# microsoft/UniVL

Measured on NVIDIA H100. Metric: video-text samples/sec, higher is better.
Workload: dtype bf16

## Files before the change

include/univl_b200.h:

```cpp
#ifndef UNIVL_B200_H_
#define UNIVL_B200_H_

#ifdef __cplusplus
extern "C" {
#endif

const char* univl_last_error_string(void);
int univl_abi_version(void);
int univl_set_reserved_sms(int n);

int univl_gemm_bf16(const void* A, long long lda, int a_mn_major, const void* B, long long ldb, int b_mn_major,
                    int M, int N, int Kc, void* out, long long ldo, int epilogue, const float* bias,
                    const void* aux_in, long long ld_aux_in, void* aux_out, long long ld_aux_out, float alpha,
                    int block_n, int split_k, void* stream);
int univl_gemm_plan(int M, int N, int Kc, int epilogue, int block_n, int split_k);

int univl_quantize_e4m3_rows(const void* x, long long ldx, void* q, long long ldq, float* scale, int M, int K,
                             void* stream);
int univl_quantize_e4m3_blocks(const float* w, long long ldw, void* q, long long ldq, float* scale, int N, int K,
                               void* stream);
int univl_gemm_fp8(const void* A, long long lda, const float* a_scale, const void* B, long long ldb,
                   const float* b_scale, int M, int N, int Kc, int epilogue, const float* bias, void* out,
                   long long ldo, float* out_scale, void* stream);

int univl_layernorm_fwd(const void* x, const void* res, const float* gamma, const float* beta, void* y, float* mean,
                        float* rstd, int rows, int cols, float eps, float p_drop, int drop_mode,
                        const unsigned long long* rng_state, unsigned long long stream_id, void* stream);
int univl_layernorm_bwd(const void* dy, const void* dy2, const void* x, const void* res, const float* gamma,
                        const float* mean, const float* rstd, void* dx_res, void* dx_dense, float* dgamma,
                        float* dbeta, float* dbias, int rows, int cols, float p_drop, int drop_mode,
                        const unsigned long long* rng_state, unsigned long long stream_id, void* stream);
int univl_layernorm_f32_fwd(const float* x, const float* gamma, const float* beta, void* y, float* mean, float* rstd,
                            int rows, int cols, float eps, void* stream);
int univl_layernorm_f32_bwd(const void* dy, const float* x, const float* gamma, const float* mean, const float* rstd,
                            float* dgamma, float* dbeta, int rows, int cols, void* stream);

int univl_embed_text_fwd(const long long* ids, const long long* type_ids, const float* word, const float* pos,
                         const float* type, const float* gamma, const float* beta, void* y, float* mean, float* rstd,
                         int n_seq, int S, int H, int vocab, float eps, float p_drop, const unsigned long long* rng_state,
                         unsigned long long stream_id, void* stream);
int univl_embed_text_bwd(const void* dy, const long long* ids, const long long* type_ids, const float* word,
                         const float* pos, const float* type, const float* gamma, const float* mean,
                         const float* rstd, float* dword, float* dpos, float* dtype, float* dgamma, float* dbeta,
                         int n_seq, int S, int H, int vocab, float p_drop, const unsigned long long* rng_state,
                         unsigned long long stream_id, void* stream);
int univl_embed_src_fwd(const void* a, const void* b, const float* pos, const float* type, const float* gamma,
                        const float* beta, void* y, float* mean, float* rstd, int Na, int Wa, int Nb, int Fb,
                        int all_pairs, int H, float eps, float p_drop, const unsigned long long* rng_state,
                        unsigned long long stream_id, void* stream);
int univl_embed_src_bwd(const void* dy, const void* a, const void* b, const float* pos, const float* type,
                        const float* gamma, const float* mean, const float* rstd, void* da, void* db, float* dpos,
                        float* dtype, float* dgamma, float* dbeta, int Na, int Wa, int Nb, int Fb, int all_pairs,
                        int H, float p_drop, const unsigned long long* rng_state, unsigned long long stream_id, void* stream);

int univl_attention_fwd(const void* q, long long ldq, const void* k, long long ldk, const void* v, long long ldv,
                        void* o, long long ldo, float* lse, const long long* mask_a, const long long* mask_b, int Wa,
                        int Fb, int Nb, int all_pairs, int n_seq, int heads, int Sq, int Sk, int causal, float scale,
                        float p_drop, const unsigned long long* rng_state, unsigned long long stream_id, void* stream);
int univl_attention_bwd(const void* q, long long ldq, const void* k, long long ldk, const void* v, long long ldv,
                        const void* o, long long ldo, const float* lse, const void* d_o, long long lddo, void* dq,
                        long long lddq, void* dk, long long lddk, void* dv, long long lddv, const long long* mask_a,
                        const long long* mask_b, int Wa, int Fb, int Nb, int all_pairs, int n_seq, int heads, int Sq,
                        int Sk, int causal, float scale, float p_drop, const unsigned long long* rng_state,
                        unsigned long long stream_id, int rng_layout, float* dbq, float* dbk, float* dbv, void* stream);
int univl_attention_long_fwd(const void* q, long long ldq, const void* k, long long ldk, const void* v, long long ldv,
                             void* o, long long ldo, float* lse, const long long* mask_a, const long long* mask_b,
                             int Wa, int Fb, int Nb, int all_pairs, int n_seq, int heads, int Sq, int Sk, int causal,
                             float scale, float p_drop, const unsigned long long* rng_state,
                             unsigned long long stream_id, void* stream);
int univl_attention_long_bwd(const void* q, long long ldq, const void* k, long long ldk, const void* v, long long ldv,
                             const void* o, long long ldo, const float* lse, const void* d_o, long long lddo, void* dq,
                             long long lddq, void* dk, long long lddk, void* dv, long long lddv,
                             const long long* mask_a, const long long* mask_b, int Wa, int Fb, int Nb, int all_pairs,
                             int n_seq, int heads, int Sq, int Sk, int causal, float scale, float p_drop,
                             const unsigned long long* rng_state, unsigned long long stream_id, int rng_layout,
                             float* dbq, float* dbk, float* dbv, void* stream);
int univl_attention_pair_fwd(const void* qa, long long ldqa, const void* ka, long long ldka, const void* va,
                             long long ldva, const void* qb, long long ldqb, const void* kb, long long ldkb,
                             const void* vb, long long ldvb, void* o, long long ldo, float* lse,
                             const long long* mask_a, const long long* mask_b, int Na, int Wa, int Nb, int Fb,
                             int heads, int Sq, float scale, void* stream);
int univl_fused_qkv_attention_supported(int n_seq, int heads, int S, int H);
int univl_fused_qkv_attention_fwd(const void* x, long long ldx, const void* wqkv, long long ldw, const float* bias,
                                  void* qkv_out, long long ld_qkv, void* o, long long ldo, float* lse,
                                  const long long* mask_a, const long long* mask_b, int Wa, int Fb, int Nb,
                                  int all_pairs, int n_seq, int heads, int S, int causal, float scale, float p_drop,
                                  const unsigned long long* rng_state, unsigned long long stream_id, void* stream);
int univl_fused_attention_bwd(const void* qkv, long long ld_qkv, const void* o, long long ldo, const float* lse,
                              const void* d_o, long long lddo, void* dqkv, long long ld_dqkv, float* dbias,
                              const long long* mask_a, const long long* mask_b, int Wa, int Fb, int Nb, int all_pairs,
                              int n_seq, int heads, int S, int causal, float scale, float p_drop,
                              const unsigned long long* rng_state, unsigned long long stream_id, void* stream);

int univl_colsum_bf16(const void* x, long long ld, float* out, int rows, int cols, void* stream);
int univl_cast_f32_to_bf16(const float* src, void* dst, long long n, void* stream);
int univl_cast_bf16_to_f32(const void* src, float* dst, long long n, void* stream);
int univl_multi_cast_f32_to_bf16(const unsigned long long* device_table, int n_tensors, int blocks_per_tensor,
                                 void* stream);
int univl_fill_f32(float* p, float value, long long n, void* stream);
int univl_rng_advance(unsigned long long* rng_state, void* stream);
int univl_gelu_fwd_bf16(const void* x, void* out, long long n, void* stream);
int univl_gelu_bwd_bf16(const void* dy, const void* pre, void* out, long long n, void* stream);
int univl_tanh_fwd_bf16(const void* x, void* out, long long n, void* stream);
int univl_tanh_bwd_bf16(const void* dy, const void* y, void* out, long long n, void* stream);
int univl_scale_f32(float* dst, const float* src, long long n, const float* gscale, void* stream);

int univl_meanpool_fwd(const void* x, const long long* mask, float* out, float* norm_out, int N, int S, int H,
                       int skip_first, int guard_zero, int l2norm, void* stream);
int univl_meanpool_bwd(const float* dy, const float* y, const float* norm, const long long* mask, void* dx, int N,
                       int S, int H, int skip_first, int guard_zero, int l2norm, void* stream);
int univl_sim_matmul_fwd(const float* t, const float* v, float* sim, int Bt, int Bv, int H, int groups, void* stream);
int univl_sim_matmul_bwd(const float* dsim, const float* t, const float* v, float* dt, float* dv, int Bt, int Bv,
                         int H, int groups, void* stream);
int univl_maxmargin_loss(const float* sim, float* loss, float* dsim, int B, float margin, int n_pair, float w_same,
                         float w_diff, int groups, void* stream);
int univl_crossen_loss(const float* sim, float* loss, float* dsim, int B, int groups, void* stream);
int univl_milnce_loss(const float* sim, float* loss, float* dsim, int batch_size, int n_pair, int groups,
                      void* stream);
int univl_softmax_xent_fwd(const float* logits, long long ld, const long long* labels, const long long* pair_mask,
                           float* lse, float* sum_count, float* loss, int T, int V, int target_mode,
                           long long ignore_index, int groups, void* stream);
int univl_softmax_xent_bwd(const float* logits, long long ld, const long long* labels, const long long* pair_mask,
                           const float* lse, const float* sum_count, const float* gscale, void* dlogits,
                           long long ld_d, int T, int V, int target_mode, long long ignore_index, int groups,
                           void* stream);
int univl_vocab_xent_workspace(int T, int V);
int univl_vocab_xent_fwd(const void* x, long long ldx, const void* w, long long ldw, const float* bias,
                         const long long* labels, float* lse, float* sum_count, float* loss, void* workspace,
                         long long workspace_bytes, int T, int V, int Kc, int groups, void* stream);
int univl_vocab_xent_bwd(const void* x, long long ldx, const void* w, long long ldw, const float* bias,
                         const long long* labels, const float* lse, const float* sum_count, const float* gscale,
                         void* dlogits, long long ld_d, int T, int V, int Kc, int groups, void* stream);
int univl_pooler_sim_fwd(const void* u, const float* w, const float* b, float* out, int N, int H, void* stream);
int univl_pooler_sim_bwd(const void* u, const float* w, const float* dout, void* du, float* dw, float* db, int N,
                         int H, void* stream);

int univl_bert_adam_step(float* p, const float* g, float* m, float* v, void* p_bf16, const void* segs, int n_chunks,
                         int n_tensors, float* scratch, long long* step, float b1, float b2, float eps,
                         float max_grad_norm, float global_clip_norm, float warmup, long long t_total,
                         float grad_scale, void* stream);
int univl_bert_adam_step_bf16grad(float* p, const void* g_bf16, float* m, float* v, void* p_bf16, const void* segs,
                                  int n_chunks, int n_tensors, float* scratch, long long* step, float b1, float b2,
                                  float eps, float max_grad_norm, float global_clip_norm, float warmup,
                                  long long t_total, float grad_scale, void* stream);

#ifdef __cplusplus
}
#endif
#endif
```

univl_b200/csrc/api.cu:

```cuda
#include "common.cuh"

#include <stdarg.h>
#include <stdio.h>
#include <stdlib.h>

namespace univl {

static thread_local char g_err[512] = "";

int set_error(int code, const char* fmt, ...) {
  va_list ap;
  va_start(ap, fmt);
  vsnprintf(g_err, sizeof(g_err), fmt, ap);
  va_end(ap);
  return code;
}

bool pdl_enabled() {
  static int v = -1;
  if (v < 0) {
    const char* e = getenv("UNIVL_PDL");
    v = (e && e[0] == '1') ? 1 : 0;
  }
  return v == 1;
}

static int g_reserved_sms = 0;

int device_sms() {
  static int sms = 0;
  if (sms == 0) {
    int dev = 0, n = 132;
    cudaGetDevice(&dev);
    cudaDeviceGetAttribute(&n, cudaDevAttrMultiProcessorCount, dev);
    sms = n;
  }
  return sms;
}

int usable_sms() {
  const int n = device_sms() - g_reserved_sms;
  return n < 8 ? 8 : n;
}

int scratch_alloc(void** p, size_t bytes, cudaStream_t st) {
  static bool pool_ready[64] = {};
  int dev = 0;
  cudaGetDevice(&dev);
  if (dev < 64 && !pool_ready[dev]) {
    cudaMemPool_t pool;
    if (cudaDeviceGetDefaultMemPool(&pool, dev) == cudaSuccess) {
      uint64_t keep = ~0ull;
      cudaMemPoolSetAttribute(pool, cudaMemPoolAttrReleaseThreshold, &keep);
    }
    pool_ready[dev] = true;
  }
  const cudaError_t e = cudaMallocAsync(p, bytes < 16 ? 16 : bytes, st);
  if (e != cudaSuccess) return set_error(UNIVL_ERR_CUDA, "scratch allocation of %zu bytes: %s", bytes, cudaGetErrorString(e));
  return UNIVL_OK;
}

__global__ void __launch_bounds__(256)
partials_reduce_kernel(const float* __restrict__ part, int nparts, long long rows, long long cols, float* __restrict__ dst,
                       long long ld) {
  const long long n = rows * cols;
  for (long long i = blockIdx.x * 256LL + threadIdx.x; i < n; i += (long long)gridDim.x * 256) {
    float t = 0.f;
    for (int k = 0; k < nparts; ++k) t += part[(long long)k * n + i];
    const long long r = i / cols, c = i - r * cols;
    dst[r * ld + c] += t;
  }
}

int partials_reduce(float* part, int nparts, long long rows, long long cols, float* dst, long long ld, cudaStream_t st) {
  const long long n = rows * cols;
  long long blocks = (n + 255) / 256;
  if (blocks > device_sms() * 8LL) blocks = device_sms() * 8LL;
  if (blocks < 1) blocks = 1;
  partials_reduce_kernel<<<(int)blocks, 256, 0, st>>>(part, nparts, rows, cols, dst, ld);
  const cudaError_t e = cudaGetLastError();
  cudaFreeAsync(part, st);
  if (e != cudaSuccess) return set_error(UNIVL_ERR_CUDA, "partials_reduce launch: %s", cudaGetErrorString(e));
  return UNIVL_OK;
}

}

extern "C" int univl_set_reserved_sms(int n) {
  if (n < 0) return univl::set_error(UNIVL_ERR_ARG, "univl_set_reserved_sms: n = %d", n);
  univl::g_reserved_sms = n;
  return UNIVL_OK;
}
extern "C" const char* univl_last_error_string() { return univl::g_err; }
extern "C" int univl_abi_version() { return 1; }
```

Baseline: 1364.

## Restructure split-K partials reduction to stage many partials through shared memory

Rewrites the partials reduction kernel so each block covers 32 output elements, with 8 warps cooperatively loading partial slices into a double-buffered shared-memory tile and warp 0 summing them. The grid is no longer capped, and loads use streaming cache hints. This targets reductions with many partials, where the old kernel ran one long serial loop per thread. The cost is extra shared-memory traffic and barriers, plus a serial sum by one warp per block, which may hurt when nparts is small. It also exposes a public C entry point for the reduction.

```diff
diff --git a/include/univl_b200.h b/include/univl_b200.h
--- a/include/univl_b200.h
+++ b/include/univl_b200.h
@@ -8,6 +8,8 @@
 const char* univl_last_error_string(void);
 int univl_abi_version(void);
 int univl_set_reserved_sms(int n);
+int univl_partials_reduce(const float* part, int nparts, long long rows, long long cols, float* dst, long long ld,
+                          void* stream);
 
 int univl_gemm_bf16(const void* A, long long lda, int a_mn_major, const void* B, long long ldb, int b_mn_major,
                     int M, int N, int Kc, void* out, long long ldo, int epilogue, const float* bias,
diff --git a/univl_b200/csrc/api.cu b/univl_b200/csrc/api.cu
--- a/univl_b200/csrc/api.cu
+++ b/univl_b200/csrc/api.cu
@@ -60,28 +60,63 @@
   return UNIVL_OK;
 }
 
-__global__ void __launch_bounds__(256)
-partials_reduce_kernel(const float* __restrict__ part, int nparts, long long rows, long long cols, float* __restrict__ dst,
+constexpr int PR_WARPS = 8;
+constexpr int PR_STAGE = 256;
+constexpr int PR_SMEM = 2 * PR_STAGE * 32 * 4;
+
+__global__ void __launch_bounds__(PR_WARPS * 32)
+partials_reduce_kernel(const float* __restrict__ part, int nparts, long long n, long long cols, float* __restrict__ dst,
                        long long ld) {
-  const long long n = rows * cols;
-  for (long long i = blockIdx.x * 256LL + threadIdx.x; i < n; i += (long long)gridDim.x * 256) {
-    float t = 0.f;
-    for (int k = 0; k < nparts; ++k) t += part[(long long)k * n + i];
-    const long long r = i / cols, c = i - r * cols;
+  extern __shared__ float pr_tile[];
+  constexpr int PER = PR_STAGE / PR_WARPS;
+  const int warp = threadIdx.x >> 5, lane = threadIdx.x & 31;
+  const long long e = blockIdx.x * 32LL + lane;
+  const bool ok = e < n;
+  const int stages = (nparts + PR_STAGE - 1) / PR_STAGE;
+  float v[PER];
+  auto load = [&](int s) {
+#pragma unroll
+    for (int i = 0; i < PER; ++i) {
+      const int k = s * PR_STAGE + i * PR_WARPS + warp;
+      v[i] = ok && k < nparts ? __ldcs(part + (long long)k * n + e) : 0.f;
+    }
+  };
+  if (stages > 0) load(0);
+  float t = 0.f;
+  for (int s = 0; s < stages; ++s) {
+    float* tile = pr_tile + (s & 1) * PR_STAGE * 32;
+#pragma unroll
+    for (int i = 0; i < PER; ++i) tile[(i * PR_WARPS + warp) * 32 + lane] = v[i];
+    __syncthreads();
+    if (s + 1 < stages) load(s + 1);
+    if (warp == 0) {
+      const int kn = nparts - s * PR_STAGE < PR_STAGE ? nparts - s * PR_STAGE : PR_STAGE;
+      for (int k = 0; k < kn; ++k) t += tile[k * 32 + lane];
+    }
+  }
+  if (warp == 0 && ok) {
+    const long long r = e / cols, c = e - r * cols;
     dst[r * ld + c] += t;
   }
 }
 
-int partials_reduce(float* part, int nparts, long long rows, long long cols, float* dst, long long ld, cudaStream_t st) {
+static int partials_reduce_launch(const float* part, int nparts, long long rows, long long cols, float* dst, long long ld,
+                                  cudaStream_t st) {
   const long long n = rows * cols;
-  long long blocks = (n + 255) / 256;
-  if (blocks > device_sms() * 8LL) blocks = device_sms() * 8LL;
-  if (blocks < 1) blocks = 1;
-  partials_reduce_kernel<<<(int)blocks, 256, 0, st>>>(part, nparts, rows, cols, dst, ld);
-  const cudaError_t e = cudaGetLastError();
-  cudaFreeAsync(part, st);
+  const long long blocks = n > 0 ? (n + 31) / 32 : 1;
+  if (blocks > 0x7fffffffLL) return set_error(UNIVL_ERR_UNSUPPORTED, "partials_reduce: %lld elements", n);
+  cudaError_t e = cudaFuncSetAttribute(partials_reduce_kernel, cudaFuncAttributeMaxDynamicSharedMemorySize, PR_SMEM);
+  if (e != cudaSuccess) return set_error(UNIVL_ERR_CUDA, "partials_reduce smem attribute: %s", cudaGetErrorString(e));
+  partials_reduce_kernel<<<(unsigned)blocks, PR_WARPS * 32, PR_SMEM, st>>>(part, nparts, n, cols, dst, ld);
+  e = cudaGetLastError();
   if (e != cudaSuccess) return set_error(UNIVL_ERR_CUDA, "partials_reduce launch: %s", cudaGetErrorString(e));
   return UNIVL_OK;
+}
+
+int partials_reduce(float* part, int nparts, long long rows, long long cols, float* dst, long long ld, cudaStream_t st) {
+  const int rc = partials_reduce_launch(part, nparts, rows, cols, dst, ld, st);
+  cudaFreeAsync(part, st);
+  return rc;
 }
 
 }
@@ -91,5 +126,11 @@
   univl::g_reserved_sms = n;
   return UNIVL_OK;
 }
+extern "C" int univl_partials_reduce(const float* part, int nparts, long long rows, long long cols, float* dst,
+                                     long long ld, void* stream) {
+  UNIVL_CHECK_ARG(part && dst && nparts >= 0 && rows >= 0 && cols > 0 && ld >= cols,
+                  "partials_reduce: bad arguments nparts=%d rows=%lld cols=%lld ld=%lld", nparts, rows, cols, ld);
+  return univl::partials_reduce_launch(part, nparts, rows, cols, dst, ld, (cudaStream_t)stream);
+}
 extern "C" const char* univl_last_error_string() { return univl::g_err; }
 extern "C" int univl_abi_version() { return 1; }
```

Measured after the change: 1445 (median of 6 runs). 1.06x the previous value.
